# ziotom78/pytracer

Measured on AMD Instinct MI355X. Metric: Mray/s (primary+shadow; rays handed to a world query) at 1280x720 per GPU, C2: 32 spheres + 1 plane, FlatRenderer, higher is better.
Workload: dtype f64; 1 GPU; C2 flat 1280x720, 32 spheres + 1 plane, S=0, every primary ray traced (dome shortcut off), fp32 RGB resident in HBM; width=1280, height=720, renderer=FlatRenderer

## Files before the change

pytracer_amd/csrc/pt_tile.h:

```cpp
struct TileCone {
  float ox, oy, oz;
  float ax, ay, az;
  float cos_t, sin_t;
  float oabs;
  bool all;
  float kx, ky, kz;
  float dmax2;
  float dmin;
  float rbeam;
  bool ortho;
};

struct ConeCam {
  float d0[3], dx[3], dy[3], apex[3];
  bool ortho;
};

PT_DEV ConeCam cone_cam(const PtKArgs &a) {
  ConeCam k;
  pt_kargs c = cold_args(a);
  for (int i = 0; i < 3; ++i) {
    k.d0[i] = c->cone_d0[i];
    k.dx[i] = c->cone_dx[i];
    k.dy[i] = c->cone_dy[i];
// ... 635 lines not shown
                                __int_as_float(__builtin_amdgcn_readlane(__float_as_int(bq.z), bit)),
                                __int_as_float(__builtin_amdgcn_readlane(__float_as_int(bq.w), bit))};
              hitable = hitable || cone_keeps(pc, b);
            }
          }
        }
        const V3 cum = dc_cum;
        if (active && !hitable) {
          store_pixel(a, pix, cum, out_f32);
          nrays += (unsigned long long)nsamp;
          nres += (unsigned long long)nsamp;
        }
        const unsigned long long todo = __ballot(active && hitable);
        if (lane == 0) {
          rmask[tile] = todo;
          rkeys[tile] = (unsigned char)__popcll(todo);
            if (todo) note_flagged(pt_queue(a), __popcll(todo));
        }
        __builtin_amdgcn_wave_barrier();
        continue;
      }
    }

    Pcg pcg;
    unsigned long long gpix = 0;
    if (S > 0) {
      pt_kargs c = cold_args(a);
      gpix = (unsigned long long)grow * c->W + pcol;
      pcg_seed_pixel(pcg, c->pcg_mode, c->s0, c->q0, gpix, nsamp);
    }
    V3 cum = {0.0, 0.0, 0.0};
    bool alive = active;
    int pix_rays = 0;
    for (int s = 0; s < nsamp; ++s) {
      if (RENDERER == PT_RENDERER_PATHTRACER && !__any(alive)) break;
      double up = 0.5, vp = 0.5;
      if (S > 0) {
        pt_kargs c = cold_args(a);
        if (c->pcg_mode == PT_PCG_SAMPLE) pcg_seed(pcg, c->s0, c->q0 + gpix * (unsigned)nsamp + (unsigned)s);
        const int sr = s / S, sc = s - sr * S;
        up = ((double)sc + pcg_float(pcg)) / (double)S;
        vp = ((double)sr + pcg_float(pcg)) / (double)S;
      }
      const Ray ray = primary_ray(a, pcol, grow, up, vp);
      PT_TSTAMP(3);
      double best_t;
      const int hit = world_query_tile<RENDERER == PT_RENDERER_ONOFF, HIER, !ORTHO>(a, ray, mbase, tpass, best_t, alive, list);
      PT_TSTAMP(4);
      if (alive) pix_rays++;
      V3 c;
      {
        pt_kargs ca = cold_args(a);
        c.x = ca->bg[0];
        c.y = ca->bg[1];
        c.z = ca->bg[2];
      }
      if (RENDERER == PT_RENDERER_ONOFF) {
        if (hit >= 0) {
          pt_kargs ca = cold_args(a);
          c.x = ca->onoff[0];
          c.y = ca->onoff[1];
          c.z = ca->onoff[2];
        }
      } else if (RENDERER == PT_RENDERER_POINTLIGHT) {
        unsigned long long shadow_rays = 0;
        c = pointlight_shade(a, ray, hit, best_t, alive, c, shadow_rays);
        pix_rays += (int)shadow_rays;
      } else if (RENDERER == PT_RENDERER_PATHTRACER) {
        if (hit >= 0) {
          pt_kargs ca = cold_args(a);
          const PtShapeAux *ax = ca->aux + hit;
          Hit h;
          h.u = 0.0;
          h.v = 0.0;
          if (ax->needs_uv) hit_details(a.recs + hit, ax, ray, best_t, h, true);
          const V3 hc = brdf_pigment(a, ax, h.u, h.v);
          const V3 em = emitted_pigment(a, ax, h.u, h.v);
          const double lum = max2(max2(hc.x, hc.y), hc.z);
          if (ca->rr <= 0 || lum > 0.0) alive = false;
          const double invN = 1.0 / (double)ca->N;
          c.x = em.x + 0.0 * invN;
          c.y = em.y + 0.0 * invN;
          c.z = em.z + 0.0 * invN;
        }
      } else {
        if (hit >= 0) {
          const PtShapeAux *ax = cold_args(a)->aux + hit;
          Hit h;
          h.u = 0.0;
          h.v = 0.0;
          if (ax->needs_uv) hit_details(a.recs + hit, ax, ray, best_t, h, true);
          const V3 p1 = brdf_pigment(a, ax, h.u, h.v);
          const V3 p2 = emitted_pigment(a, ax, h.u, h.v);
          c.x = p1.x + p2.x;
          c.y = p1.y + p2.y;
          c.z = p1.z + p2.z;
        }
      }
      if (S > 0) {
        cum.x = cum.x + c.x;
        cum.y = cum.y + c.y;
        cum.z = cum.z + c.z;
      } else {
        cum = c;
      }
      PT_TSTAMP(5);
    }
    if (S > 0) {
      const double k = 1.0 / (double)(S * S);
      cum.x = cum.x * k;
      cum.y = cum.y * k;
      cum.z = cum.z * k;
    }
    if (alive) {
      store_pixel(a, pix, cum, out_f32);
      nrays += (unsigned long long)pix_rays;
    }
    if (RENDERER == PT_RENDERER_PATHTRACER) {
      const unsigned long long todo = __ballot(active && !alive);
      if (lane == 0) {
        rmask[tile] = todo;
        rkeys[tile] = (unsigned char)__popcll(todo);
        if (todo) note_flagged(pt_queue(a), __popcll(todo));
      }
    }
    __builtin_amdgcn_wave_barrier();
    PT_TSTAMP(6);
   }
   }
  }
#ifdef PT_DEBUG_TIME
  if (RENDERER != PT_RENDERER_PATHTRACER && (threadIdx.x & 63) == 0 && (blockIdx.x & 63) == 0)
    for (int q = 0; q < 8; ++q) atomicAdd(pt_queue(a) + 1 + q, tsum[q]);
  pt_dbg_flush();
#endif
  add_ray_count(a, nrays, count_base, nres);
}

struct Hit4 {
  double best_t[4];
  int best[4];
};

template <bool ANYHIT>
PT_DEV void sphere_roots1(const PtKArgs &a, int slot, bool active, double tmin, double ox, double oy, double oz, double dx,
                          double dy, double dz, double aa, double cc, double &best_t, int &best) {
  const double tmax = INFINITY;
  PT_SPHERE_ROOTS(slot);
}

#ifndef PT_TILE4_WAVES
#define PT_TILE4_WAVES 4
#endif
template <int RENDERER, bool SLDS = false>
__global__ __launch_bounds__(PT_BLOCK) __attribute__((amdgpu_waves_per_eu(PT_TILE4_WAVES, 8))) void pt_tile4_kernel(const PtKArgs a) {
  constexpr int NPX = 4;
  constexpr int TH = 16;
  constexpr bool ANYHIT = RENDERER == PT_RENDERER_ONOFF;
#ifdef PT_DEBUG_TIME
  unsigned long long tsum[8] = {0, 0, 0, 0, 0, 0, 0, 0}, tprev = __builtin_amdgcn_s_memtime();
#define PT_T4(k) do { const unsigned long long tn = __builtin_amdgcn_s_memtime(); tsum[k] += tn - tprev; tprev = tn; } while (0)
#else
#define PT_T4(k) do { } while (0)
#endif
  int W, rows_local, npass;
  bool dome_on, out_f32;
  {
    pt_kargs c = cold_args(a);
    out_f32 = c->out_f32 != 0;
    W = c->W;
    rows_local = c->rows_local;
    npass = c->npass;
    dome_on = c->dome_shortcut != 0;
  }
  const int lane = threadIdx.x & 63, wib = threadIdx.x >> 6;
  const int tx = blockIdx.x * 2 + (wib & 1), ty = blockIdx.y * 2 + (wib >> 1);
  unsigned long long nrays = 0, nres = 0;
  const bool valid = tx * 16 < W && ty * TH < rows_local;
  if (SLDS) {
    const unsigned long long *src = (const unsigned long long *)a.recs;
    for (int k = threadIdx.x; k < a.n_shapes * 16; k += PT_BLOCK) pt_lds_masks[k] = src[k];
    src = (const unsigned long long *)a.aux;
    for (int k = threadIdx.x; k < a.n_shapes * 32; k += PT_BLOCK) pt_lds_masks[a.n_shapes * 16 + k] = src[k];
    __syncthreads();
  }
  if (valid) {
    const int lr0 = ty * TH, lr1 = (lr0 + TH - 1 < rows_local) ? lr0 + TH - 1 : rows_local - 1;
    const int gr0 = global_row(a, lr0);
    const float4 b_first = a.bounds[lane < a.n_shapes ? lane : 0];
    PT_T4(0);
    const TileCone tc = tile_cone(a, tx * 16, (tx * 16 + 16 < W) ? tx * 16 + 16 : W, gr0, gr0 + (lr1 - lr0));
    PT_T4(1);
    unsigned long long masks[4] = {0ULL, 0ULL, 0ULL, 0ULL};
    int nsurv = 0, only = 0;
#pragma unroll
    for (int p = 0; p < 4; ++p) {
      if (p < npass) {
        const int slot = p * 64 + lane;
        bool keep = false;
        float4 b = {0.0f, 0.0f, 0.0f, -1.0f};
        if (slot < a.n_shapes) b = p == 0 ? b_first : a.bounds[slot];
        const bool isplane = slot >= a.n_spheres && slot < a.n_shapes;
        if (slot < a.n_spheres) keep = cone_keeps(tc, b);
        if (__any(isplane)) {
          const bool pk = plane_keeps(tc, b, isplane);
          if (isplane) keep = pk;
        }
        const unsigned long long m = __ballot(keep);
        masks[p] = m;
        nsurv += __popcll(m);
        if (m) only = p * 64 + (__ffsll((long long)m) - 1);
      }
    }
    PT_T4(2);
    const int colA = tx * 16 + (lane & 7), colB = colA + 8;
    const int lrowA = lr0 + (lane >> 3), lrowB = lrowA + 8;
    const bool okcA = colA < W, okcB = colB < W, okrA = lrowA < rows_local, okrB = lrowB < rows_local;
    const bool act[4] = {okcA && okrA, okcB && okrA, okcA && okrB, okcB && okrB};
    const int ccA = okcA ? colA : W - 1, ccB = okcB ? colB : W - 1;
    const int crA = okrA ? lrowA : rows_local - 1, crB = okrB ? lrowB : rows_local - 1;
    const long long pix[4] = {(long long)crA * W + ccA, (long long)crA * W + ccB, (long long)crB * W + ccA, (long long)crB * W + ccB};
    bool done = false;
    if (dome_on && nsurv == 1 && only < a.n_spheres) {
      only = __builtin_amdgcn_readfirstlane(only);
      pt_kargs ca = cold_args(a);
      const PtShapeAux *ax = ca->aux + only;
      const float fro2 = (float)PT_KD(&a.recs[only])[13];
      const double hc = (only < a.n_diag) ? PT_KD(&a.hoist_diag[only])[6] : PT_KD(&a.hoist[only])[3];
      if (ax->needs_uv == 0 && hc < -0.5 && fro2 * tc.dmax2 < 1e6f && tc.dmin > 1e-6f && !tc.all) {
        V3 c;
        if (RENDERER == PT_RENDERER_ONOFF) {
          c.x = ca->onoff[0];
          c.y = ca->onoff[1];
          c.z = ca->onoff[2];
        } else {
          const V3 p1 = brdf_pigment(a, ax, 0.0, 0.0), p2 = emitted_pigment(a, ax, 0.0, 0.0);
          c.x = p1.x + p2.x;
          c.y = p1.y + p2.y;
          c.z = p1.z + p2.z;
        }
#pragma unroll
        for (int k = 0; k < NPX; ++k)
          if (act[k]) {
            store_pixel(a, pix[k], c, out_f32);
            nrays += 1ULL;
            nres += 1ULL;
          }
        done = true;
      }
    }
    PT_T4(3);
    if (!done) {
      V3 org, dir[4];
      double bgx, bgy, bgz;
      {
        pt_kargs c = cold_args(a);
        const double dist = c->cam_dist, aspect = c->cam_aspect;
        const double Wd = (double)c->W, Hd = (double)c->H;
        const int growA = gr0 + (crA - lr0), growB = gr0 + (crB - lr0);
        const double uA = ((double)ccA + 0.5) / Wd, uB = ((double)ccB + 0.5) / Wd;
        const double vA = 1.0 - ((double)growA + 0.5) / Hd, vB = 1.0 - ((double)growB + 0.5) / Hd;
        const double dyA = (1.0 - 2.0 * uA) * aspect, dyB = (1.0 - 2.0 * uB) * aspect;
        const double dzA = 2.0 * vA - 1.0, dzB = 2.0 * vB - 1.0;
        const double m0 = c->cam_m[0], m1 = c->cam_m[1], m2 = c->cam_m[2], m3 = c->cam_m[3];
        const double m4 = c->cam_m[4], m5 = c->cam_m[5], m6 = c->cam_m[6], m7 = c->cam_m[7];
        const double m8 = c->cam_m[8], m9 = c->cam_m[9], m10 = c->cam_m[10], m11 = c->cam_m[11];
        const double xA = dist * m0 + dyA * m1, xB = dist * m0 + dyB * m1;
        const double yA = dist * m4 + dyA * m5, yB = dist * m4 + dyB * m5;
        const double zA = dist * m8 + dyA * m9, zB = dist * m8 + dyB * m9;
        dir[0] = {xA + dzA * m2, yA + dzA * m6, zA + dzA * m10};
        dir[1] = {xB + dzA * m2, yB + dzA * m6, zB + dzA * m10};
        dir[2] = {xA + dzB * m2, yA + dzB * m6, zA + dzB * m10};
        dir[3] = {xB + dzB * m2, yB + dzB * m6, zB + dzB * m10};
        const double ox_ = -dist, oy_ = 0.0, oz_ = 0.0;
        org.x = ox_ * m0 + oy_ * m1 + oz_ * m2 + m3;
        org.y = ox_ * m4 + oy_ * m5 + oz_ * m6 + m7;
        org.z = ox_ * m8 + oy_ * m9 + oz_ * m10 + m11;
        bgx = c->bg[0];
        bgy = c->bg[1];
        bgz = c->bg[2];
      }
      PT_T4(4);
      const double tmin = 1.0e-5;
      Hit4 h4;
      bool fast = true;
#pragma unroll
      for (int k = 0; k < NPX; ++k) {
        h4.best_t[k] = INFINITY;
        h4.best[k] = -1;
        Ray rk;
        rk.o = org;
        rk.d = dir[k];
        rk.tmin = tmin;
        fast = fast && wave_guard<true>(rk, act[k]).fast;
      }
      const int nd = a.n_diag, ns = a.n_spheres;
      bool all_hit = false;
#pragma unroll
      for (int p = 0; p < 4; ++p) {
        unsigned long long mask = masks[p];
        while (mask && !all_hit) {
          const int slot = p * 64 + (__ffsll((long long)mask) - 1);
          mask &= mask - 1;
          if (slot < ns) {
            if (slot < nd && fast) {
              pt_kdouble h = PT_KD(&a.hoist_diag[slot]);
              const double s0 = h[0], s1 = h[1], s2 = h[2], ox = h[3], oy = h[4], oz = h[5], cc = h[6];
#pragma unroll
              for (int k = 0; k < NPX; ++k) {
                const double dx = dir[k].x * s0, dy = dir[k].y * s1, dz = dir[k].z * s2;
                const double aa = dx * dx + dy * dy + dz * dz;
                sphere_roots1<ANYHIT>(a, slot, act[k], tmin, ox, oy, oz, dx, dy, dz, aa, cc, h4.best_t[k], h4.best[k]);
              }
            } else {
              pt_kdouble m = PT_KD(a.recs[slot].invm);
              pt_kdouble h = PT_KD(&a.hoist[slot]);
              const double ox = h[0], oy = h[1], oz = h[2], cc = h[3];
#pragma unroll
              for (int k = 0; k < NPX; ++k) {
                const double dx = dir[k].x * m[0] + dir[k].y * m[1] + dir[k].z * m[2];
                const double dy = dir[k].x * m[4] + dir[k].y * m[5] + dir[k].z * m[6];
                const double dz = dir[k].x * m[8] + dir[k].y * m[9] + dir[k].z * m[10];
                const double aa = dx * dx + dy * dy + dz * dz;
                sphere_roots1<ANYHIT>(a, slot, act[k], tmin, ox, oy, oz, dx, dy, dz, aa, cc, h4.best_t[k], h4.best[k]);
              }
            }
          } else {
            pt_kdouble m = PT_KD(a.recs[slot].invm);
            const double oz = PT_KD(&a.hoist[slot])[2];
            const double tmax = INFINITY;
#pragma unroll
            for (int k = 0; k < NPX; ++k) {
              const double dz = dir[k].x * m[8] + dir[k].y * m[9] + dir[k].z * m[10];
              const bool active = act[k];
              double &best_t = h4.best_t[k];
              int &best = h4.best[k];
              PT_PLANE_HIT(slot);
            }
          }
          if (ANYHIT) {
            const bool open = (act[0] && h4.best[0] < 0) || (act[1] && h4.best[1] < 0) || (act[2] && h4.best[2] < 0) ||
                              (act[3] && h4.best[3] < 0);
            all_hit = __ballot(open) == 0ULL;
          }
        }
      }
      PT_T4(5);
#pragma unroll
      for (int k = 0; k < NPX; ++k) {
        V3 c = {bgx, bgy, bgz};
        const int hit = h4.best[k];
        if (RENDERER == PT_RENDERER_ONOFF) {
          if (hit >= 0) {
            pt_kargs ca = cold_args(a);
            c.x = ca->onoff[0];
            c.y = ca->onoff[1];
            c.z = ca->onoff[2];
          }
        } else if (hit >= 0) {
          Hit h;
          h.u = 0.0;
          h.v = 0.0;
          Ray rk;
          rk.o = org;
          rk.d = dir[k];
          rk.tmin = tmin;
          V3 p1, p2;
          if constexpr (SLDS) {
            const pt_lds_rec rec = (pt_lds_rec)(const void *)pt_lds_f64 + hit;
            const pt_lds_aux ax = (pt_lds_aux)(const void *)(pt_lds_f64 + a.n_shapes * 16) + hit;
            if (ax->needs_uv) {
              hit_details(rec, ax, rk, h4.best_t[k], h, true);
              p1 = brdf_pigment(a, ax, h.u, h.v);
              p2 = emitted_pigment(a, ax, h.u, h.v);
              c.x = p1.x + p2.x;
              c.y = p1.y + p2.y;
              c.z = p1.z + p2.z;
            } else {
              c.x = ax->pig_c2[0];
              c.y = ax->pig_c2[1];
              c.z = ax->pig_c2[2];
            }
          } else {
            const PtShapeAux *ax = cold_args(a)->aux + hit;
            if (ax->needs_uv) {
              hit_details(a.recs + hit, ax, rk, h4.best_t[k], h, true);
              p1 = brdf_pigment(a, ax, h.u, h.v);
              p2 = emitted_pigment(a, ax, h.u, h.v);
              c.x = p1.x + p2.x;
              c.y = p1.y + p2.y;
              c.z = p1.z + p2.z;
            } else {
              c.x = ax->pig_c2[0];
              c.y = ax->pig_c2[1];
              c.z = ax->pig_c2[2];
            }
          }
        }
        PT_T4(6);
        if (act[k]) {
          store_pixel(a, pix[k], c, out_f32);
          nrays += 1ULL;
        }
        PT_T4(7);
      }
    }
  }
#ifdef PT_DEBUG_TIME
#ifdef PT_DEBUG_HEAVY
  {
    unsigned long long tot_ = 0;
    for (int q = 0; q < 8; ++q) tot_ += tsum[q];
    if ((threadIdx.x & 63) == 0 && ((blockIdx.y * gridDim.x + blockIdx.x) & 3) == 0 && tot_ > PT_DEBUG_HEAVY)
      for (int q = 0; q < 8; ++q) atomicAdd(pt_queue(a) + 1 + q, tsum[q]);
  }
#else
  if ((threadIdx.x & 63) == 0 && ((blockIdx.y * gridDim.x + blockIdx.x) & 15) == 0)
    for (int q = 0; q < 8; ++q) atomicAdd(pt_queue(a) + 1 + q, tsum[q]);
#endif
  if ((threadIdx.x & 63) == 0) {
    const int wv = (blockIdx.y * gridDim.x + blockIdx.x) * 4 + (int)(threadIdx.x >> 6);
    if (wv < PT_UNITLOG_LEN) {
      unsigned long long tot_ = 0;
      for (int q = 0; q < 8; ++q) tot_ += tsum[q];
      pt_unitlog[wv * 8] = tot_;
      pt_unitlog[wv * 8 + 1] = tsum[0] + tsum[1] + tsum[2] + tsum[3];
      pt_unitlog[wv * 8 + 2] = __builtin_amdgcn_s_memtime();
    }
  }
  if ((threadIdx.x & 63) == 0 && ((blockIdx.y * gridDim.x + blockIdx.x) & 15) == 0) {
    unsigned long long tot = 0;
    for (int q = 0; q < 8; ++q) tot += tsum[q];
    atomicMax(pt_queue(a) + 12, tot);
    if (tot > 16384ULL) atomicAdd(pt_queue(a) + 13, 1ULL);
    if (tot > 24576ULL) atomicAdd(pt_queue(a) + 14, 1ULL);
    if (tot > 32768ULL) atomicAdd(pt_queue(a) + 15, 1ULL);
  }
#endif
  add_ray_count(a, nrays, 0, nres, blockIdx.y * gridDim.x + blockIdx.x);
}
```

pytracer_amd/csrc/ptrace.hip:

```cpp
#include <hip/hip_runtime.h>
#include <hip/hip_ext.h>

#include <algorithm>
#include <atomic>
#include <cmath>
#include <cstdarg>
#include <cstdio>
#include <cstdlib>
#include <cstring>
#include <new>
#include <vector>

#include "../../include/ptrace.h"
#include "../../include/ptrace_debug.h"
#include "pt_kernels.h"
#include "pt_layout.h"
#include "pt_plan.h"
#include "pt_scene_build.h"
#include "pt_hits_plan.h"
#include "pt_post.h"

#define PT_VERSION ((1 << 16) | 7)


// ... 508 lines not shown
  a.frame_doubles = pl.frame_doubles;
  a.diag_lds = pl.diag_lds;
  a.grid_occ_lds = pl.grid_occ_lds;
  a.scene_lds = pl.scene_lds;
  a.nthreads = pl.nthreads;
  a.block_h = pl.block_h;
  s->stats.grid = pl.grid;
  s->stats.block = PT_BLOCK;
  s->stats.lds_bytes = 0;
  s->stats.kernel = pl.kernel;
  const int n_count_slots = pl.grid + pl.grid_first + pl.grid_q;

  if (s->count_rays) {
    size_t have = (size_t)s->ray_partials_n * 2;
    int rc = ensure(&s->ray_partials, &have, (size_t)n_count_slots * 2, st);
    s->ray_partials_n = (int)(have / 2);
    if (rc) return rc;
    a.ray_counter = s->ray_partials;
  }

  if (pl.hoist && !(s->hoist_valid && s->hoist_stream == st && memcmp(&s->hoist_cam, cam, sizeof(pt_camera)) == 0)) {
    V3 o = {-cam->screen_distance, 0.0, 0.0};
    V3 w;
    w.x = o.x * cam->m[0] + o.y * cam->m[1] + o.z * cam->m[2] + cam->m[3];
    w.y = o.x * cam->m[4] + o.y * cam->m[5] + o.z * cam->m[6] + cam->m[7];
    w.z = o.x * cam->m[8] + o.y * cam->m[9] + o.z * cam->m[10] + cam->m[11];
    hipLaunchKernelGGL(pt_prep_hoist, dim3((a.n_shapes + 255) / 256), dim3(256), 0, st, a.recs, s->hoist,
                       s->hoist_diag, a.n_shapes, a.n_diag, w);
    s->hoist_cam = *cam;
    s->hoist_valid = true;
    s->hoist_stream = st;
  }

  if (pl.zero_frame) {
    HIP_TRY(hipEventRecord(s->ev0, st));
    HIP_TRY(hipMemsetAsync(out_dev, 0, pt_output_bytes(p), st));
    HIP_TRY(hipEventRecord(s->ev1, st));
    if (s->count_rays) {
      HIP_TRY(hipMemsetAsync(s->ray_counter, 0, 2 * sizeof(unsigned long long), st));
      HIP_TRY(hipMemcpyAsync(s->ray_counter_host, s->ray_counter, 2 * sizeof(unsigned long long),
                             hipMemcpyDeviceToHost, st));
      HIP_TRY(hipEventRecord(s->ev_count, st));
      s->count_pending = true;
    }
    return PT_OK;
  }
  if (p->renderer == PT_RENDERER_PATHTRACER) {
    a.qpar = s->queue_parity;
    s->queue_last = s->queue + (size_t)a.qpar * PT_QUEUE_WORDS;
    if (!s->queue_clean) HIP_TRY(hipMemsetAsync(s->queue_last, 0, PT_QUEUE_WORDS * sizeof(unsigned long long), st));
    s->queue_clean = false;
    a.p_max_path = pl.p_max_path;
    a.s_min_path = pl.s_min_path;
    size_t have = s->ws_bytes / sizeof(double);
    int rc = ensure(&s->ws, &have, (pl.ws_bytes + sizeof(double) - 1) / sizeof(double), st);
    s->ws_bytes = have * sizeof(double);
    if (rc) return rc;
    a.ws = s->ws;
  }

  if (pl.path_tiled) {
    int rc = ensure(&s->region_keys, &s->region_keys_cap, (size_t)pl.nregions, st);
    if (!rc) rc = ensure(&s->region_mask, &s->region_mask_cap, (size_t)pl.nregions, st);
    if (!rc) rc = ensure(&s->units, &s->units_cap, (size_t)pl.units_need, st);
    if (rc) return rc;
    a.units = s->units;
    a.region_keys = s->region_keys;
    a.region_mask = s->region_mask;
    a.spec_draws = pl.spec_draws;
    a.tree_jump_lds = pl.tree_jump_lds;
    if (pl.q_alt) {
      rc = ensure(&s->handover, &s->handover_doubles, pl.handover_doubles, st);
      if (rc) return rc;
      rc = ensure(&s->units_handed, &s->units_handed_n, (size_t)pl.handover_cap, st);
      if (rc) return rc;
    }
    a.handover = s->handover;
    a.units_handed = s->units_handed;
    a.handover_cap = pl.q_alt ? pl.handover_cap : 0;
    s->last_handover_cap = a.handover_cap;
    a.q_budget = 0;
    a.q_tail_budget = 0;
    a.q_few_lanes = 0;
    a.dbg_trace_unit = (int)tn.trace_unit;
    a.dome_slot = -1;
    if (!pl.ortho && tn.pixel_dome) {
      const double ox = -cam->screen_distance * cam->m[0] + cam->m[3], oy = -cam->screen_distance * cam->m[4] + cam->m[7],
                   oz = -cam->screen_distance * cam->m[8] + cam->m[11];
      double best = -0.5;
      for (const auto &dc : s->sh->dome_cands) {
        const double *m = dc.invm;
        const double px = ox * m[0] + oy * m[1] + oz * m[2] + m[3], py = ox * m[4] + oy * m[5] + oz * m[6] + m[7],
                     pz = ox * m[8] + oy * m[9] + oz * m[10] + m[11];
        const double c = px * px + py * py + pz * pz - 1.0;
        if (c < best) {
          best = c;
          a.dome_slot = dc.slot;
        }
      }
    }
  }
  if (pl.hier) {
    int rc = ensure(&s->cell_list, &s->cell_list_cap, (size_t)pl.ncells * pl.cell_stride, st);
    if (!rc) rc = ensure(&s->cell_count, &s->cell_count_cap, (size_t)pl.ncells, st);
    if (rc) return rc;
    a.cell_list = s->cell_list;
    a.cell_count = s->cell_count;
    a.cells_x = pl.cells_x;
    a.cell_stride = pl.cell_stride;
  }
  a.cold = s->args.dev;
  if (int rc = refresh_cold(s->args, a, st)) return rc;
  const void *main_fn = nullptr;
  const bool prof = s->timing && s->profiling && (size_t)(2 * s->prof_used + 1) < s->prof.size();
  const hipEvent_t ev_a = s->timing ? (prof ? s->prof[2 * s->prof_used] : s->ev0) : nullptr;
  const hipEvent_t ev_b = s->timing ? (prof ? s->prof[2 * s->prof_used + 1] : s->ev1) : nullptr;
  bool ev_started = false;
  const int R = p->renderer;
#ifdef PT_DEBUG_TIME
  if (pl.tile4 || ((pl.tile || pl.path_tiled) && R != PT_RENDERER_PATHTRACER)) {
    s->queue_last = s->queue;
    HIP_TRY(hipMemsetAsync(s->queue, 0, 16 * sizeof(unsigned long long), st));
    if (s->queue_parity == 0) s->queue_clean = false;
  }
#endif
  if (hits_channels >= 0) {
    const size_t lds = hits_cull ? pl.lds_tile : 0;
    s->stats.lds_bytes = (int)lds;
    if (hits_cull && pl.hier) {
      if (pl.cell_chunk_len > PT_CELL_CHUNK) return fail(PT_ERR_INVALID, "internal: cell chunk exceeds its LDS staging");
      HIP_TRY(hipMemsetAsync(s->cell_count, 0, (size_t)pl.ncells * sizeof(int), st));
      PT_LAUNCH(pt_cell_kernel, pl.cell_groups * pl.cell_chunks, 0, false, a, pl.cell_chunks, pl.cell_chunk_len);
    }
    if (!hits_cull && pl.ortho)
      PT_LAUNCH((pt_hits_kernel<false, true, false>), pl.grid, lds, true, a, hits_channels);
    else if (!hits_cull)
      PT_LAUNCH((pt_hits_kernel<false, false, false>), pl.grid, lds, true, a, hits_channels);
    else if (pl.tile_mode == PT_TILE_HIER)
      PT_LAUNCH((pt_hits_kernel<true, false, true>), pl.grid, lds, true, a, hits_channels);
    else if (pl.tile_mode == PT_TILE_ORTHO)
      PT_LAUNCH((pt_hits_kernel<false, true, true>), pl.grid, lds, true, a, hits_channels);
    else
      PT_LAUNCH((pt_hits_kernel<false, false, true>), pl.grid, lds, true, a, hits_channels);
  } else if (pl.tile4) {
    s->stats.lds_bytes = (int)pl.lds_main;
    const dim3 grid4(pl.grid4_x, pl.grid4_y, 1);
#define PT_LAUNCH4(R_, L_)                                                                                                  \
  do {                                                                                                                      \
    main_fn = (const void *)pt_tile4_kernel<R_, L_>;                                                                        \
    hipExtLaunchKernelGGL((pt_tile4_kernel<R_, L_>), grid4, dim3(PT_BLOCK), pl.lds_main, st, ev_a, ev_b, 0, a);             \
  } while (0)
    if (R == PT_RENDERER_ONOFF)
      PT_LAUNCH4(PT_RENDERER_ONOFF, false);
    else if (pl.t4lds)
      PT_LAUNCH4(PT_RENDERER_FLAT, true);
    else
      PT_LAUNCH4(PT_RENDERER_FLAT, false);
#undef PT_LAUNCH4
  } else if (pl.tile || pl.path_tiled) {
    const size_t lds = pl.lds_tile;
    s->stats.lds_bytes = (int)lds;
    const int tgrid = pl.path_tiled ? pl.grid_first : pl.grid;
    const bool last = !pl.path_tiled;
    const int pgrid = pl.path_tiled ? pl.grid : 0;
    if (pl.hier) {
      if (pl.cell_chunk_len > PT_CELL_CHUNK) return fail(PT_ERR_INVALID, "internal: cell chunk exceeds its LDS staging");
      HIP_TRY(hipMemsetAsync(s->cell_count, 0, (size_t)pl.ncells * sizeof(int), st));
      PT_LAUNCH(pt_cell_kernel, pl.cell_groups * pl.cell_chunks, 0, false, a, pl.cell_chunks, pl.cell_chunk_len);
    }
#define PT_TILE_MODES(R_, W_)                                                                              \
  do {                                                                                                     \
    if (pl.tile_mode == PT_TILE_HIER)                                                                      \
      PT_LAUNCH((pt_tile_kernel<R_, W_, true>), tgrid, lds, last, a, pgrid);                               \
    else if (pl.tile_mode == PT_TILE_ORTHO)                                                                \
      PT_LAUNCH((pt_tile_kernel<R_, W_, false, true>), tgrid, lds, last, a, pgrid);                        \
    else                                                                                                   \
      PT_LAUNCH((pt_tile_kernel<R_, W_, false>), tgrid, lds, last, a, pgrid);                              \
  } while (0)
    if (R == PT_RENDERER_ONOFF)
      PT_TILE_MODES(PT_RENDERER_ONOFF, 4);
    else if (R == PT_RENDERER_FLAT)
      PT_TILE_MODES(PT_RENDERER_FLAT, 4);
    else if (R == PT_RENDERER_POINTLIGHT)
      PT_TILE_MODES(PT_RENDERER_POINTLIGHT, PT_WAVES_POINTLIGHT);
    else if (pl.tile_mode == PT_TILE_BLOCKS)
      PT_LAUNCH((pt_tile_kernel<PT_RENDERER_PATHTRACER, 4, false, false, true>), tgrid, lds, last, a, pgrid);
    else
      PT_TILE_MODES(PT_RENDERER_PATHTRACER, 4);
#undef PT_TILE_MODES
    if (pl.path_tiled) {
      if (pl.tree)
        hipLaunchKernelGGL(pt_unit_scatter, dim3(pl.grid_scatter), dim3(PT_SCATTER_BLOCK), 0, st, s->region_keys, s->region_mask, pl.nregions,
                           s->units, (int)s->units_cap, s->queue_last, (long long)1 << 60, 64, 1, pl.q_min, pl.q_budget_per_flagged, pl.q_budget_min);
      else
        hipLaunchKernelGGL(pt_unit_scatter, dim3(pl.grid_scatter), dim3(PT_SCATTER_BLOCK), 0, st, s->region_keys, s->region_mask, pl.nregions,
                           s->units, (int)s->units_cap, s->queue_last, pl.lanes_cap, pl.nsamp, (long long)pl.min_rounds);
      if (pl.q_alt) {
        PtKArgs aq = a;
        aq.cold = s->args2.dev;
        aq.nthreads = pl.grid_q * PT_BLOCK;
        aq.frame_doubles = 20;
        aq.p_max_path = pl.q_p_max_path;
        aq.s_min_path = pl.q_s_min_path;
        aq.count_base = pl.grid + pl.grid_first;
        aq.q_budget = pl.q_budget;
        aq.q_tail_budget = pl.q_tail_budget;
        aq.q_few_lanes = pl.q_few_lanes;
        aq.scene_lds = -1;
        aq.grid_occ_lds = -1;
        aq.diag_lds = pl.q_diag_lds;
        aq.ws = s->ws;
        if (int rc = refresh_cold(s->args2, aq, st)) return rc;
#define PT_ALT(K_)                                              \
  do {                                                          \
    HIP_TRY(path_lds_limit((const void *)(K_), pl.lds_q));      \
    PT_LAUNCH((K_), pl.grid_q, pl.lds_q, false, aq);            \
  } while (0)
        switch (pl.alt) {
          case PT_ALT_FLAGGED_LEAN_LDS: PT_ALT((pt_path_flagged_kernel<1, 1>)); break;
          case PT_ALT_FLAGGED_LEAN_SPLIT: PT_ALT((pt_path_flagged_kernel<1, 2>)); break;
          case PT_ALT_FLAGGED_SPLIT: PT_ALT((pt_path_flagged_kernel<0, 2>)); break;
          default: PT_ALT((pt_path_flagged_kernel<0, 1>)); break;
        }
#undef PT_ALT
      }
      const bool last2 = true;
#define PT_SECOND(K_)                                               \
  do {                                                              \
    HIP_TRY(path_lds_limit((const void *)(K_), pl.lds_main));       \
    PT_LAUNCH((K_), pl.grid, pl.lds_main, last2, a);                \
  } while (0)
      switch (pl.second) {
        case PT_SECOND_TREE_LEAN: PT_SECOND((pt_path_tree_kernel<true>)); break;
        case PT_SECOND_TREE_LEAN_SCENE: PT_SECOND((pt_path_tree_kernel<true, true>)); break;
        case PT_SECOND_TREE: PT_SECOND((pt_path_tree_kernel<false>)); break;
        case PT_SECOND_REGIONS_LDS_SCENE_LEAN: PT_SECOND((pt_path_regions_kernel<true, true, 1>)); break;
        case PT_SECOND_REGIONS_LDS_SCENE: PT_SECOND((pt_path_regions_kernel<true, true>)); break;
        case PT_SECOND_REGIONS_LDS_NOGRID: PT_SECOND((pt_path_regions_kernel<true, false, 2>)); break;
        case PT_SECOND_REGIONS_LDS: PT_SECOND((pt_path_regions_kernel<true>)); break;
        default: PT_SECOND((pt_path_regions_kernel<false>)); break;
      }
#undef PT_SECOND
      if (pl.q_alt && (s->timing || s->count_rays || prof)) {
        HIP_TRY(hipMemcpyAsync(s->ray_counter_host + 2, s->queue_last + PT_Q_CHOICE, sizeof(unsigned long long), hipMemcpyDeviceToHost, st));
        s->choice_pending = true;
      }
    }
  } else if (R == PT_RENDERER_PATHTRACER) {
    PT_LAUNCH(pt_path_kernel, pl.grid, 0, true, a);
  } else {
#define PT_SIMPLE(R_)                                                              \
  do {                                                                             \
    if (pl.simple_hoist)                                                           \
      PT_LAUNCH((pt_simple_kernel<R_, true>), pl.grid, 0, true, a);                \
    else                                                                           \
      PT_LAUNCH((pt_simple_kernel<R_, false>), pl.grid, 0, true, a);               \
  } while (0)
    if (R == PT_RENDERER_ONOFF)
      PT_SIMPLE(PT_RENDERER_ONOFF);
    else if (R == PT_RENDERER_FLAT)
      PT_SIMPLE(PT_RENDERER_FLAT);
    else
      PT_SIMPLE(PT_RENDERER_POINTLIGHT);
#undef PT_SIMPLE
  }
  HIP_TRY(hipGetLastError());
  if (p->renderer == PT_RENDERER_PATHTRACER) {
    s->queue_parity ^= 1;
    s->queue_clean = true;
  }
  if (main_fn) {
    static std::vector<std::pair<const void *, int>> known;
    int regs = -1;
    for (const auto &kv : known)
      if (kv.first == main_fn) regs = kv.second;
    if (regs < 0) {
      hipFuncAttributes fa;
      regs = hipFuncGetAttributes(&fa, main_fn) == hipSuccess ? fa.numRegs : 0;
      (void)hipGetLastError();
      known.push_back({main_fn, regs});
    }
    s->stats.vgprs = regs;
  }
  if (prof) {
    s->prof_used++;
    s->stats_valid = false;
  } else if (s->timing) {
    s->stats_valid = true;
  } else {
    s->stats_valid = false;
  }
  if (s->count_rays) {
    hipLaunchKernelGGL(pt_sum_counts, dim3(1), dim3(256), 0, st, s->ray_partials, n_count_slots, s->ray_counter);
    HIP_TRY(hipMemcpyAsync(s->ray_counter_host, s->ray_counter, 2 * sizeof(unsigned long long),
                           hipMemcpyDeviceToHost, st));
    HIP_TRY(hipEventRecord(s->ev_count, st));
    s->count_pending = true;
  } else if (s->choice_pending) {
    HIP_TRY(hipEventRecord(s->ev_count, st));
  }
  return PT_OK;
}

static int fold_stats(pt_scene *s) {
  if (!s->pending) return PT_OK;
  float ms = 0.f;
  if (s->stats_valid) HIP_TRY(hipEventSynchronize(s->pending_copy ? s->ev2 : s->ev1));
  if (!s->stats_valid) {
    HIP_TRY(hipStreamSynchronize(s->last_stream));
// ... 831 lines not shown
```

Baseline: 66060 Mray/s.

## Stage scene tables into LDS asynchronously and defer the barrier to shading

The shape-record and aux tables are now copied into LDS with direct global-to-LDS async loads issued at kernel start. The barrier moves from before culling and tracing to just before shading, so the copy overlaps with cone culling and intersection. Camera and launch parameters are preloaded and pinned to scalar registers, and the row-mapping helper is inlined. This adds host-side alignment and size checks and a hard cap on the scene image that can be staged; scenes larger than the cap now fail to launch.

```diff
diff --git a/pytracer_amd/csrc/pt_tile.h b/pytracer_amd/csrc/pt_tile.h
--- a/pytracer_amd/csrc/pt_tile.h
+++ b/pytracer_amd/csrc/pt_tile.h
@@ -811,6 +811,8 @@
 #ifndef PT_TILE4_WAVES
 #define PT_TILE4_WAVES 4
 #endif
+#define PT_TILE4_STAGE_ROUNDS 6
+#define PT_PIN_SGPR(x) asm volatile("" : "+s"(x))
 template <int RENDERER, bool SLDS = false>
 __global__ __launch_bounds__(PT_BLOCK) __attribute__((amdgpu_waves_per_eu(PT_TILE4_WAVES, 8))) void pt_tile4_kernel(const PtKArgs a) {
   constexpr int NPX = 4;
@@ -822,33 +824,73 @@
 #else
 #define PT_T4(k) do { } while (0)
 #endif
-  int W, rows_local, npass;
-  bool dome_on, out_f32;
-  {
-    pt_kargs c = cold_args(a);
-    out_f32 = c->out_f32 != 0;
-    W = c->W;
-    rows_local = c->rows_local;
-    npass = c->npass;
-    dome_on = c->dome_shortcut != 0;
-  }
-  const int lane = threadIdx.x & 63, wib = threadIdx.x >> 6;
+  const int lane = threadIdx.x & 63, wib = __builtin_amdgcn_readfirstlane((int)(threadIdx.x >> 6));
+  int W, rows_local, npass, n_ranks, row_block, rank, dome_sw, f32_sw, cam_kind;
+  ConeCam cam;
+  pt_kargs c0 = cold_args(a);
+  W = c0->W;
+  rows_local = c0->rows_local;
+  npass = c0->npass;
+  dome_sw = c0->dome_shortcut;
+  f32_sw = c0->out_f32;
+  n_ranks = c0->n_ranks;
+  row_block = c0->row_block;
+  rank = c0->rank;
+  cam_kind = c0->cam_kind;
+  for (int i = 0; i < 3; ++i) {
+    cam.d0[i] = c0->cone_d0[i];
+    cam.dx[i] = c0->cone_dx[i];
+    cam.dy[i] = c0->cone_dy[i];
+    cam.apex[i] = c0->cone_apex[i];
+  }
+  const float4 b_first = a.bounds[lane < a.n_shapes ? lane : 0];
+  if constexpr (SLDS) {
+    const int nrec = a.n_shapes * (int)sizeof(PtShapeRec), nimg = nrec + a.n_shapes * (int)sizeof(PtShapeAux);
+    const char *src_rec = (const char *)a.recs, *src_aux = (const char *)a.aux - nrec;
+#pragma unroll
+    for (int r = 0; r < PT_TILE4_STAGE_ROUNDS; ++r) {
+      const int cbase = (r * (PT_BLOCK / 64) + wib) * 1024, b = cbase + lane * 16;
+      if (b < nimg)
+        __builtin_amdgcn_global_load_lds((const __attribute__((address_space(1))) void *)((b < nrec ? src_rec : src_aux) + b),
+                                         (__attribute__((address_space(3))) void *)((char *)pt_lds_masks + cbase), 16, 0, 0);
+    }
+  }
+  PT_PIN_SGPR(f32_sw);
+  PT_PIN_SGPR(n_ranks);
+  PT_PIN_SGPR(row_block);
+  PT_PIN_SGPR(rank);
+  PT_PIN_SGPR(W);
+  PT_PIN_SGPR(rows_local);
+  PT_PIN_SGPR(npass);
+  PT_PIN_SGPR(dome_sw);
+  PT_PIN_SGPR(cam_kind);
+  for (int i = 0; i < 3; ++i) {
+    PT_PIN_SGPR(cam.d0[i]);
+    PT_PIN_SGPR(cam.dx[i]);
+    PT_PIN_SGPR(cam.dy[i]);
+    PT_PIN_SGPR(cam.apex[i]);
+  }
+  cam.ortho = cam_kind != PT_CAMERA_PERSPECTIVE;
+  const bool dome_on = dome_sw != 0, out_f32 = f32_sw != 0;
   const int tx = blockIdx.x * 2 + (wib & 1), ty = blockIdx.y * 2 + (wib >> 1);
   unsigned long long nrays = 0, nres = 0;
   const bool valid = tx * 16 < W && ty * TH < rows_local;
-  if (SLDS) {
-    const unsigned long long *src = (const unsigned long long *)a.recs;
-    for (int k = threadIdx.x; k < a.n_shapes * 16; k += PT_BLOCK) pt_lds_masks[k] = src[k];
-    src = (const unsigned long long *)a.aux;
-    for (int k = threadIdx.x; k < a.n_shapes * 32; k += PT_BLOCK) pt_lds_masks[a.n_shapes * 16 + k] = src[k];
-    __syncthreads();
-  }
+  bool shade = false;
+  bool act[4];
+  long long pix[4];
+  V3 org, dir[4];
+  double bgx, bgy, bgz;
+  Hit4 h4;
+  const double tmin = 1.0e-5;
   if (valid) {
     const int lr0 = ty * TH, lr1 = (lr0 + TH - 1 < rows_local) ? lr0 + TH - 1 : rows_local - 1;
-    const int gr0 = global_row(a, lr0);
-    const float4 b_first = a.bounds[lane < a.n_shapes ? lane : 0];
+    int gr0 = lr0;
+    if (n_ranks != 1) {
+      const int blk = lr0 / row_block;
+      gr0 = (blk * n_ranks + rank) * row_block + (lr0 - blk * row_block);
+    }
     PT_T4(0);
-    const TileCone tc = tile_cone(a, tx * 16, (tx * 16 + 16 < W) ? tx * 16 + 16 : W, gr0, gr0 + (lr1 - lr0));
+    const TileCone tc = tile_cone(cam, tx * 16, (tx * 16 + 16 < W) ? tx * 16 + 16 : W, gr0, gr0 + (lr1 - lr0));
     PT_T4(1);
     unsigned long long masks[4] = {0ULL, 0ULL, 0ULL, 0ULL};
     int nsurv = 0, only = 0;
@@ -875,10 +917,16 @@
     const int colA = tx * 16 + (lane & 7), colB = colA + 8;
     const int lrowA = lr0 + (lane >> 3), lrowB = lrowA + 8;
     const bool okcA = colA < W, okcB = colB < W, okrA = lrowA < rows_local, okrB = lrowB < rows_local;
-    const bool act[4] = {okcA && okrA, okcB && okrA, okcA && okrB, okcB && okrB};
+    act[0] = okcA && okrA;
+    act[1] = okcB && okrA;
+    act[2] = okcA && okrB;
+    act[3] = okcB && okrB;
     const int ccA = okcA ? colA : W - 1, ccB = okcB ? colB : W - 1;
     const int crA = okrA ? lrowA : rows_local - 1, crB = okrB ? lrowB : rows_local - 1;
-    const long long pix[4] = {(long long)crA * W + ccA, (long long)crA * W + ccB, (long long)crB * W + ccA, (long long)crB * W + ccB};
+    pix[0] = (long long)crA * W + ccA;
+    pix[1] = (long long)crA * W + ccB;
+    pix[2] = (long long)crB * W + ccA;
+    pix[3] = (long long)crB * W + ccB;
     bool done = false;
     if (dome_on && nsurv == 1 && only < a.n_spheres) {
       only = __builtin_amdgcn_readfirstlane(only);
@@ -910,8 +958,6 @@
     }
     PT_T4(3);
     if (!done) {
-      V3 org, dir[4];
-      double bgx, bgy, bgz;
       {
         pt_kargs c = cold_args(a);
         const double dist = c->cam_dist, aspect = c->cam_aspect;
@@ -940,8 +986,6 @@
         bgz = c->bg[2];
       }
       PT_T4(4);
-      const double tmin = 1.0e-5;
-      Hit4 h4;
       bool fast = true;
 #pragma unroll
       for (int k = 0; k < NPX; ++k) {
@@ -1004,65 +1048,69 @@
           }
         }
       }
-      PT_T4(5);
-#pragma unroll
-      for (int k = 0; k < NPX; ++k) {
-        V3 c = {bgx, bgy, bgz};
-        const int hit = h4.best[k];
-        if (RENDERER == PT_RENDERER_ONOFF) {
-          if (hit >= 0) {
-            pt_kargs ca = cold_args(a);
-            c.x = ca->onoff[0];
-            c.y = ca->onoff[1];
-            c.z = ca->onoff[2];
+      shade = true;
+    }
+  }
+  if constexpr (SLDS) __syncthreads();
+  if (valid) PT_T4(5);
+  if (shade) {
+#pragma unroll
+    for (int k = 0; k < NPX; ++k) {
+      V3 c = {bgx, bgy, bgz};
+      const int hit = h4.best[k];
+      if (RENDERER == PT_RENDERER_ONOFF) {
+        if (hit >= 0) {
+          pt_kargs ca = cold_args(a);
+          c.x = ca->onoff[0];
+          c.y = ca->onoff[1];
+          c.z = ca->onoff[2];
+        }
+      } else if (hit >= 0) {
+        Hit h;
+        h.u = 0.0;
+        h.v = 0.0;
+        Ray rk;
+        rk.o = org;
+        rk.d = dir[k];
+        rk.tmin = tmin;
+        V3 p1, p2;
+        if constexpr (SLDS) {
+          const pt_lds_rec rec = (pt_lds_rec)(const void *)pt_lds_f64 + hit;
+          const pt_lds_aux ax = (pt_lds_aux)(const void *)(pt_lds_f64 + a.n_shapes * 16) + hit;
+          if (ax->needs_uv) {
+            hit_details(rec, ax, rk, h4.best_t[k], h, true);
+            p1 = brdf_pigment(a, ax, h.u, h.v);
+            p2 = emitted_pigment(a, ax, h.u, h.v);
+            c.x = p1.x + p2.x;
+            c.y = p1.y + p2.y;
+            c.z = p1.z + p2.z;
+          } else {
+            c.x = ax->pig_c2[0];
+            c.y = ax->pig_c2[1];
+            c.z = ax->pig_c2[2];
           }
-        } else if (hit >= 0) {
-          Hit h;
-          h.u = 0.0;
-          h.v = 0.0;
-          Ray rk;
-          rk.o = org;
-          rk.d = dir[k];
-          rk.tmin = tmin;
-          V3 p1, p2;
-          if constexpr (SLDS) {
-            const pt_lds_rec rec = (pt_lds_rec)(const void *)pt_lds_f64 + hit;
-            const pt_lds_aux ax = (pt_lds_aux)(const void *)(pt_lds_f64 + a.n_shapes * 16) + hit;
-            if (ax->needs_uv) {
-              hit_details(rec, ax, rk, h4.best_t[k], h, true);
-              p1 = brdf_pigment(a, ax, h.u, h.v);
-              p2 = emitted_pigment(a, ax, h.u, h.v);
-              c.x = p1.x + p2.x;
-              c.y = p1.y + p2.y;
-              c.z = p1.z + p2.z;
-            } else {
-              c.x = ax->pig_c2[0];
-              c.y = ax->pig_c2[1];
-              c.z = ax->pig_c2[2];
-            }
+        } else {
+          const PtShapeAux *ax = cold_args(a)->aux + hit;
+          if (ax->needs_uv) {
+            hit_details(a.recs + hit, ax, rk, h4.best_t[k], h, true);
+            p1 = brdf_pigment(a, ax, h.u, h.v);
+            p2 = emitted_pigment(a, ax, h.u, h.v);
+            c.x = p1.x + p2.x;
+            c.y = p1.y + p2.y;
+            c.z = p1.z + p2.z;
           } else {
-            const PtShapeAux *ax = cold_args(a)->aux + hit;
-            if (ax->needs_uv) {
-              hit_details(a.recs + hit, ax, rk, h4.best_t[k], h, true);
-              p1 = brdf_pigment(a, ax, h.u, h.v);
-              p2 = emitted_pigment(a, ax, h.u, h.v);
-              c.x = p1.x + p2.x;
-              c.y = p1.y + p2.y;
-              c.z = p1.z + p2.z;
-            } else {
-              c.x = ax->pig_c2[0];
-              c.y = ax->pig_c2[1];
-              c.z = ax->pig_c2[2];
-            }
+            c.x = ax->pig_c2[0];
+            c.y = ax->pig_c2[1];
+            c.z = ax->pig_c2[2];
           }
         }
-        PT_T4(6);
-        if (act[k]) {
-          store_pixel(a, pix[k], c, out_f32);
-          nrays += 1ULL;
-        }
-        PT_T4(7);
-      }
+      }
+      PT_T4(6);
+      if (act[k]) {
+        store_pixel(a, pix[k], c, out_f32);
+        nrays += 1ULL;
+      }
+      PT_T4(7);
     }
   }
 #ifdef PT_DEBUG_TIME
diff --git a/pytracer_amd/csrc/ptrace.hip b/pytracer_amd/csrc/ptrace.hip
--- a/pytracer_amd/csrc/ptrace.hip
+++ b/pytracer_amd/csrc/ptrace.hip
@@ -684,9 +684,19 @@
   } while (0)
     if (R == PT_RENDERER_ONOFF)
       PT_LAUNCH4(PT_RENDERER_ONOFF, false);
-    else if (pl.t4lds)
+    else if (pl.t4lds) {
+      static int static_lds = -1;
+      if (static_lds < 0) {
+        hipFuncAttributes fa;
+        HIP_TRY(hipFuncGetAttributes(&fa, (const void *)pt_tile4_kernel<PT_RENDERER_FLAT, true>));
+        static_lds = (int)fa.sharedSizeBytes;
+      }
+      if ((((uintptr_t)a.recs | (uintptr_t)a.aux) & 15) != 0 || (static_lds & 15) != 0)
+        return fail(PT_ERR_INVALID, "internal: pt_tile4_kernel<FLAT, LDS> needs 16-byte aligned shape tables and LDS");
+      if (pl.lds_main > (size_t)PT_TILE4_STAGE_ROUNDS * (PT_BLOCK / 64) * 1024)
+        return fail(PT_ERR_INVALID, "internal: scene image exceeds pt_tile4_kernel's staging copy");
       PT_LAUNCH4(PT_RENDERER_FLAT, true);
-    else
+    } else
       PT_LAUNCH4(PT_RENDERER_FLAT, false);
 #undef PT_LAUNCH4
   } else if (pl.tile || pl.path_tiled) {
```

After: 68720 Mray/s (median of 6 runs). 4.0% higher.
